# DeepGraphLearning/RNNLogic

Measured on AMD Instinct MI355X. Metric: queries/sec PredictorPlus forward, FB15k-237, 1/2/4/8 GPU; MRR parity, higher is better.
Workload: dtype fp32; 1 GPU; FB15k-237 test split: 1514 batches, 40932 queries, sharded over 1 rank(s) by the reference evaluate()'s DistributedSampler; PredictorPlus(lstm,3,16,sum) + RotatE(D=1000,gamma=9); rnnlogic_rules.txt (131883 rules, L<=3); seeded synthetic train graph and RotatE tables; batch_size=32, parallelism=dp1 (test batches sharded, KG replicated), batches_per_rank=1514

## Files before the change

### include/rnnlogic_hip.h

```cpp
#ifndef RNNLOGIC_HIP_H
#define RNNLOGIC_HIP_H

#include <stddef.h>
#include <stdint.h>

#ifdef __cplusplus
extern "C" {
#endif

#define RNNL_OK 0
#define RNNL_ERR_INVALID 1
#define RNNL_ERR_HIP 2
#define RNNL_ERR_OVERFLOW 3
#define RNNL_ERR_NOMEM 4
#define RNNL_ERR_INTERNAL 5
#define RNNL_ERR_RANGE 6

#define RNNL_AGG_SUM 0
#define RNNL_AGG_PNA 1

#define RNNL_FEATURE_ADD 0
#define RNNL_FEATURE_NONE 1

typedef struct rnnl_graph_s *rnnl_graph;
// ... 85 lines not shown
                             int32_t workgroups, int32_t deferred, void *stream);
int rnnl_forward_status(void *workspace, void *stream);
int rnnl_forward_status_totals(void *workspace, void *stream, int64_t *totals);
int rnnl_forward_header_bytes(size_t *bytes);
int rnnl_forward_status_host(const void *header, int64_t *totals);
#define RNNL_FLAG_MIXED 1
int rnnl_forward_status_flags(void *workspace, void *stream, int64_t *totals, uint32_t *flags);
int rnnl_forward_flags_host(const void *header, uint32_t *flags);
int rnnl_forward_host_info(rnnl_graph g, int32_t *out);
int rnnl_ground(rnnl_graph g, rnnl_rules r, const int64_t *all_h, const int64_t *all_r,
                const int64_t *edges_to_remove, int32_t n_queries, int32_t *n_cand, void *workspace,
                size_t workspace_bytes, int32_t capacity_scale, void *stream);
int rnnl_ground_export_candidates(void *workspace, int32_t n_queries, int32_t capacity_scale, const int32_t *n_cand,
                                  const int64_t *cand_off, int32_t *out_t, int32_t *out_nent, void *stream);
int rnnl_ground_export_entries(void *workspace, int32_t n_queries, int32_t capacity_scale, const int32_t *n_cand,
                               const int64_t *ent_off, int32_t *out_node, int32_t *out_count, void *stream);
int rnnl_debug_profile(void *dev_counters);
int rnnl_debug_clock(void *dev_counters);

int rnnl_debug_capacity(int64_t frontier_base, int64_t contrib_base, int64_t pool_per_query);
int rnnl_debug_sort_bits(int32_t bits);
int rnnl_debug_pair_memo(int32_t on);
int rnnl_debug_dedupe(int32_t min_rows);

int rnnl_linear_node_weights_size(rnnl_rules r, size_t *bytes);
int rnnl_linear_node_weights(rnnl_rules r, const float *rule_weights, int32_t n_rules, void *node_w, void *stream);
int rnnl_predictor_forward(rnnl_graph g, rnnl_rules r, const void *node_w, int32_t feature, const int64_t *all_h,
                           const int64_t *all_r, const int64_t *edges_to_remove, int32_t n_queries, float *score,
                           uint8_t *mask, int32_t *n_cand, void *workspace, size_t workspace_bytes,
                           int32_t capacity_scale, void *stream);
int rnnl_predictor_ground(rnnl_graph g, rnnl_rules r, const int64_t *all_h, const int64_t *all_r,
                          const int64_t *edges_to_remove, int32_t n_queries, int32_t *n_cand, void *workspace,
                          size_t workspace_bytes, int32_t capacity_scale, void *stream);
int rnnl_predictor_score(rnnl_graph g, rnnl_rules r, const void *node_w, int32_t feature, const int64_t *all_h,
                         const int64_t *all_r, int32_t n_queries, float *score, uint8_t *mask, int32_t *n_cand,
                         void *workspace, size_t workspace_bytes, int32_t capacity_scale, void *stream);
int rnnl_predictor_rule_stats(void *workspace, int32_t n_queries, int32_t capacity_scale, const int32_t *n_cand,
                              rnnl_rules r, const int64_t *all_r, const int64_t *all_t, int32_t ld, int64_t *pos,
                              int64_t *tot, void *stream);
int rnnl_predictor_backward(void *workspace, int32_t n_queries, int32_t capacity_scale, const int32_t *n_cand,
                            rnnl_rules r, const int64_t *all_r, int32_t n_entities, const float *grad_score,
                            int32_t ld, double *grad_node, void *stream);

int rnnl_fill_rows(const float *row, int32_t n_queries, int32_t n_entities, float *score, void *stream);
int rnnl_fill_value(float value, int64_t n, float *score, void *stream);

// ... 151 lines not shown
```

### rnnlogic_amd/_native.py

```python
import ctypes
import functools
import os
import subprocess

HERE = os.path.dirname(os.path.abspath(__file__))
LIB_PATH = os.path.join(HERE, "_build", "librnnlogic_hip.so")

RNNL_OK, RNNL_ERR_INVALID, RNNL_ERR_HIP, RNNL_ERR_OVERFLOW, RNNL_ERR_NOMEM, RNNL_ERR_INTERNAL, RNNL_ERR_RANGE = \
    0, 1, 2, 3, 4, 5, 6
AGG_SUM, AGG_PNA = 0, 1
FEATURE_ADD, FEATURE_NONE = 0, 1
ROTATE_DIRECT, ROTATE_MFMA = 0, 1
FLAG_MIXED = 1
ERR_COUNT_WIDTH, ERR_NODE_RANGE, ERR_ACC_RANGE = 8, 16, 32
TOPK_MAX = 1024
KGE_TAIL, KGE_HEAD = 0, 1

_P = ctypes.c_void_p
_I32 = ctypes.c_int32
_I64 = ctypes.c_int64
_F32 = ctypes.c_float

SIGNATURES = [
    ("rnnl_last_error", ctypes.c_char_p, []),
# ... 36 lines not shown
    ("rnnl_forward_host_info", ctypes.c_int, [_P, _P]),
    ("rnnl_forward_header_bytes", ctypes.c_int, [_P]),
    ("rnnl_forward_status_host", ctypes.c_int, [_P, _P]),
    ("rnnl_forward_status_flags", ctypes.c_int, [_P, _P, _P, _P]),
    ("rnnl_forward_flags_host", ctypes.c_int, [_P, _P]),
    ("rnnl_ground", ctypes.c_int, [_P, _P, _P, _P, _P, _I32, _P, _P, ctypes.c_size_t, _I32, _P]),
    ("rnnl_ground_export_candidates", ctypes.c_int, [_P, _I32, _I32, _P, _P, _P, _P, _P]),
    ("rnnl_ground_export_entries", ctypes.c_int, [_P, _I32, _I32, _P, _P, _P, _P, _P]),
    ("rnnl_linear_node_weights_size", ctypes.c_int, [_P, _P]),
    ("rnnl_linear_node_weights", ctypes.c_int, [_P, _P, _I32, _P, _P]),
    ("rnnl_predictor_forward", ctypes.c_int,
     [_P, _P, _P, _I32, _P, _P, _P, _I32, _P, _P, _P, _P, ctypes.c_size_t, _I32, _P]),
    ("rnnl_predictor_ground", ctypes.c_int, [_P, _P, _P, _P, _P, _I32, _P, _P, ctypes.c_size_t, _I32, _P]),
    ("rnnl_predictor_score", ctypes.c_int,
     [_P, _P, _P, _I32, _P, _P, _I32, _P, _P, _P, _P, ctypes.c_size_t, _I32, _P]),
    ("rnnl_predictor_rule_stats", ctypes.c_int, [_P, _I32, _I32, _P, _P, _P, _P, _I32, _P, _P, _P]),
    ("rnnl_predictor_backward", ctypes.c_int, [_P, _I32, _I32, _P, _P, _P, _I32, _P, _I32, _P, _P]),
    ("rnnl_debug_profile", ctypes.c_int, [_P]),
    ("rnnl_debug_clock", ctypes.c_int, [_P]),
    ("rnnl_debug_capacity", ctypes.c_int, [_I64, _I64, _I64]),
    ("rnnl_debug_sort_bits", ctypes.c_int, [_I32]),
    ("rnnl_debug_pair_memo", ctypes.c_int, [_I32]),
    ("rnnl_debug_dedupe", ctypes.c_int, [_I32]),
    ("rnnl_fill_rows", ctypes.c_int, [_P, _I32, _I32, _P, _P]),
    ("rnnl_fill_value", ctypes.c_int, [_F32, _I64, _P, _P]),
    ("rnnl_rotate_table_sizes", ctypes.c_int, [_I32, _I32, _I32, _I32, _P, _P]),
    ("rnnl_rotate_entity_table", ctypes.c_int, [_P, _I32, _I32, _I32, _P, _P]),
    ("rnnl_rotate_relation_table", ctypes.c_int, [_P, _I32, _I32, _F32, _P, _P]),
    ("rnnl_rotate_workspace_size", ctypes.c_int, [_I32, _I32, _I32, _I32, _P]),
    ("rnnl_multi_hot", ctypes.c_int, [_P, _P, _P, _I64, _P, _I32, _I32, _P, _P]),
    ("rnnl_train_batch", ctypes.c_int,
     [_P, _I64, _I32, _P, _P, _P, _I64, _P, _P, _I64, _I32, _P, _P, _P, _P, _P, _P]),
    ("rnnl_filter_flags", ctypes.c_int, [_P, _P, _P, _I64, _P, _I32, _I32, _P, _P]),
    ("rnnl_filtered_ranks", ctypes.c_int, [_P, _P, _P, _P, _I32, _I32, _P, _P, _P]),
    ("rnnl_topk_rows", ctypes.c_int, [_P, _P, _P, _P, _I32, _I32, _I32, _P, _P, _P, _P]),
    ("rnnl_miner_create", ctypes.c_int, [_P, _I64, _I32, _I32, _P]),
    ("rnnl_miner_destroy", ctypes.c_int, [_P]),
    ("rnnl_rule_search", ctypes.c_int, [_P, _I32, _P, _I64, _P, _I64, _P, _P]),
    ("rnnl_miner_set_rules", ctypes.c_int, [_P, _P, _P, _P, _P]),
    ("rnnl_miner_ground_count", ctypes.c_int, [_P, _P, _I64, _I64, _P, _I64, _P, _P, _P]),
    ("rnnl_miner_ground_fill", ctypes.c_int, [_P, _P, _I64, _I64, _P, _I64, _P, _P, _P, _I64, _P, _P]),
    ("rnnl_miner_learn", ctypes.c_int,
     [_P, _P, _I64, _I64, _P, _I64, _P, _P, _P, ctypes.c_double, ctypes.c_double, ctypes.c_double, _I32, _P]),
    ("rnnl_miner_h_score", ctypes.c_int,
     [_P, _P, _I64, _I64, _P, _I64, _P, _P, _P, _I32, ctypes.c_double, ctypes.c_double, _P]),
    ("rnnl_miner_read", ctypes.c_int, [_P, _P, _P, _P]),
# ... 129 lines not shown
```

### rnnlogic_amd/csrc/fwd.h

```cpp
#pragma once
#include <hip/hip_runtime.h>

#include <algorithm>
#include <cstdint>

#include "internal.h"

namespace rnnl {

constexpr int BS = 256;
constexpr int GBS = 256;
constexpr int SOLO_GBS = 512;
constexpr int HBITS = 12;
constexpr int HCAP = 1 << HBITS;
constexpr int OCC_CAP = 1024;
constexpr int WBITS = 11;
constexpr int WIN = 1 << WBITS;
constexpr int MAXE_BITS = 19;
constexpr int SORT_WINS = 256;
constexpr int MAX_SBITS = MAXE_BITS - 8;
static_assert((SORT_WINS << MAX_SBITS) == (1 << MAXE_BITS), "SORT_WINS windows of 2^MAX_SBITS entities hold 2^MAXE_BITS");
static_assert((1 << MAX_SBITS) <= WIN, "a sort window must fit the dense pass's direct map");
constexpr int HB = WIN;
constexpr int HB_LOAD = HB * 3 / 4;
// ... 51 lines not shown
  int32_t sbits;
  float *score;
  uint8_t *mask;
  int32_t *n_cand;
  uint64_t *digest;
  unsigned char *ws;
  int64_t fcap, pcap, pool_cap;
  int32_t nslots;
  unsigned char *slots;
  int64_t *q_base;
  float *q_scale;
  const int32_t *order;
  int32_t atomic_out;
  const int32_t *row_of;
  int4 *cand;
  int2 *bent;
  float *memo;
  unsigned long long *ptab, *ptab_region;
  int32_t psbits, pbr, pbo, pbc, pbc3;
  int2 *chunks;
  int64_t chunk_cap;
  unsigned long long *prof;
};

extern unsigned long long *g_prof;

__device__ __forceinline__ uint64_t mix64(uint64_t x) {
  x += 0x9E3779B97F4A7C15ULL;
  x = (x ^ (x >> 30)) * 0xBF58476D1CE4E5B9ULL;
  x = (x ^ (x >> 27)) * 0x94D049BB133111EBULL;
  return x ^ (x >> 31);
}

__device__ __forceinline__ uint32_t hash32(uint32_t k) { return k * 2654435761u; }

__device__ __forceinline__ int64_t score_index(const KParams &p, int q, int t) {
  return (int64_t)(p.row_of ? p.row_of[q] : q) * p.g.E + t;
}

struct Ent {
  uint32_t k, c;
};

struct Slot {
  Ent *f0;
  int64_t fcap;
// ... 170 lines not shown
    trailer[1] = (unsigned)shift;
    trailer[2] = bad ? 1u : 0u;
  }
  return shift;
}

__device__ __forceinline__ void next_chunks(unsigned int *ctr, long long nchunks, int k, unsigned &c, unsigned &cend) {
  const unsigned long long stat = (unsigned long long)gridDim.x * (BS / 64) * k;
  if (cend == 0u) {
    c = (blockIdx.x * (BS / 64) + (threadIdx.x >> 6)) * (unsigned)k;
  } else if ((long long)stat >= nchunks) {
    c = (unsigned)nchunks;
  } else {
    if ((threadIdx.x & 63) == 0) c = (unsigned)stat + atomicAdd(ctr, (unsigned)k);
    c = __builtin_amdgcn_readfirstlane(c);
  }
  cend = c + (unsigned)k;
}

extern bool g_pair_memo;
void launch_chunk_list(const KParams &p, hipStream_t st);
void launch_ground(const KParams &p, int agg, hipStream_t st, int grid = 0);
void launch_score(const KParams &p, const RulesDev &rl, hipStream_t st, int grid);
int setup_params(const char *who, rnnl_graph g, rnnl_rules r, const int64_t *all_h, const int64_t *all_r,
                 const int64_t *etr, int32_t nq, int32_t *n_cand, void *ws, size_t ws_bytes, int32_t scale,
                 KParams &p);
void set_score_params(KParams &p, const rnnl_predictor_params *pp, float *score, uint8_t *mask, uint64_t *digest);
bool bad_params(const rnnl_predictor_params *pp, const float *score);
KParams export_params(void *ws, int32_t nq, int32_t scale, const int32_t *n_cand);
void plan_enqueue(const Plan &pl, hipStream_t st);
void replicate_enqueue(const Plan &pl, int E, float *score, int32_t *n_cand, hipStream_t st);

}
```

### rnnlogic_amd/csrc/ground.hip

```cpp
#include <hip/hip_runtime.h>

#include <cstdlib>
#include <map>
#include <cstring>
#include <string>

#include "fwd.h"
#include "hostside.h"

namespace rnnl {

unsigned long long *g_prof = nullptr;
int64_t g_fcap_base = FCAP_BASE, g_pcap_base = PCAP_BASE, g_pool_per_query = POOL_PER_QUERY;
int g_sort_bits = -1;

template <int G>
struct __align__(16) SmemT {
  union {
    struct {
      int key[HCAP];
      uint32_t val[HCAP];
    } a;
    struct {
      int map[WIN];
// ... 1252 lines not shown
                              const int64_t *all_r, const int64_t *etr, int32_t nq, int32_t *n_cand, void *ws,
                              size_t ws_bytes, int32_t scale, int32_t workgroups, void *stream) {
  if (aggregator != RNNL_AGG_SUM && aggregator != RNNL_AGG_PNA) {
    set_error("rnnl_predictorplus_ground: bad aggregator");
    return RNNL_ERR_INVALID;
  }
  KParams p;
  if (int rc = setup_params("rnnl_predictorplus_ground", g, r, all_h, all_r, etr, nq, n_cand, ws, ws_bytes, scale,
                            p))
    return rc;
  hipStream_t st = (hipStream_t)stream;
  RNNL_HIP_CHECK(hipMemsetAsync(ws, 0, HDR_WORDS_BYTES, st));
  if (nq == 0) return RNNL_OK;
  p.agg = aggregator;
  launch_ground(p, aggregator, st, workgroups);
  RNNL_HIP_CHECK(hipGetLastError());
  return RNNL_OK;
}

static int score_rows(rnnl_graph g, rnnl_rules r, const rnnl_predictor_params *pp, const int64_t *all_h,
                      const int64_t *all_r, int32_t nq, float *score, uint8_t *mask, int32_t *n_cand,
                      uint64_t *digest, void *ws, size_t ws_bytes, int32_t scale, int32_t workgroups,
                      int32_t deferred, const int32_t *row_of, void *stream) {
  if (bad_params(pp, score) || !n_cand || (deferred != 0 && deferred != 2) ||
      (deferred == 2 && (mask || pp->feature != RNNL_FEATURE_ADD))) {
    set_error("rnnl_predictorplus_score: bad arguments");
    return RNNL_ERR_INVALID;
  }
  KParams p;
  if (int rc = setup_params("rnnl_predictorplus_score", g, r, all_h, all_r, nullptr, nq, n_cand, ws, ws_bytes,
                            scale, p))
    return rc;
  if (nq == 0) return RNNL_OK;
  set_score_params(p, pp, score, mask, digest);
  p.atomic_out = deferred == 2;
  p.row_of = row_of;
  hipStream_t st = (hipStream_t)stream;
  launch_score(p, r->d, st, workgroups);
  RNNL_HIP_CHECK(hipGetLastError());
  return RNNL_OK;
}

int rnnl_predictorplus_score(rnnl_graph g, rnnl_rules r, const rnnl_predictor_params *pp, const int64_t *all_h,
                             const int64_t *all_r, int32_t nq, float *score, uint8_t *mask, int32_t *n_cand,
                             uint64_t *digest, void *ws, size_t ws_bytes, int32_t scale, int32_t workgroups,
                             int32_t deferred, void *stream) {
  return score_rows(g, r, pp, all_h, all_r, nq, score, mask, n_cand, digest, ws, ws_bytes, scale, workgroups, deferred,
                    nullptr, stream);
}

int rnnl_ground(rnnl_graph g, rnnl_rules r, const int64_t *all_h, const int64_t *all_r, const int64_t *etr,
                int32_t nq, int32_t *n_cand, void *ws, size_t ws_bytes, int32_t scale, void *stream) {
  KParams p;
  if (int rc = setup_params("rnnl_ground", g, r, all_h, all_r, etr, nq, n_cand, ws, ws_bytes, scale, p)) return rc;
  hipStream_t st = (hipStream_t)stream;
  RNNL_HIP_CHECK(hipMemsetAsync(ws, 0, HDR_WORDS_BYTES, st));
  if (nq == 0) return RNNL_OK;
  p.agg = RNNL_AGG_SUM;
  launch_ground(p, RNNL_AGG_SUM, st);
  RNNL_HIP_CHECK(hipGetLastError());
  return RNNL_OK;
}

int rnnl_ground_export_candidates(void *ws, int32_t nq, int32_t scale, const int32_t *n_cand,
                                  const int64_t *cand_off, int32_t *out_t, int32_t *out_nent, void *stream) {
  if (!ws || nq < 0 || scale < 1 || !n_cand || !cand_off || !out_t || !out_nent) {
    set_error("rnnl_ground_export_candidates: bad arguments");
    return RNNL_ERR_INVALID;
  }
// ... 13 lines not shown
  }
  if (nq == 0) return RNNL_OK;
  const KParams p = export_params(ws, nq, scale, n_cand);
  hipLaunchKernelGGL(export_entries_kernel, dim3((unsigned)std::min<int64_t>(nq, 4096)), dim3(EXP_BS), 0,
                     (hipStream_t)stream, p, ent_off, out_node, out_count);
  RNNL_HIP_CHECK(hipGetLastError());
  return RNNL_OK;
}

int rnnl_debug_pair_memo(int32_t on) {
  g_pair_memo = on != 0;
  return RNNL_OK;
}

constexpr int32_t DEDUPE_MIN_ROWS = 512;
static int32_t g_dedupe_min = DEDUPE_MIN_ROWS;

int rnnl_debug_dedupe(int32_t min_rows) {
  if (min_rows < -1) {
    set_error("rnnl_debug_dedupe: need min_rows >= 0 (0: off), or -1 for the default");
    return RNNL_ERR_INVALID;
  }
  g_dedupe_min = min_rows < 0 ? DEDUPE_MIN_ROWS : min_rows;
  return RNNL_OK;
}

int rnnl_debug_sort_bits(int32_t bits) {
  g_sort_bits = bits;
  return RNNL_OK;
}

int rnnl_debug_profile(void *dev_counters) {
  g_prof = static_cast<unsigned long long *>(dev_counters);
  return RNNL_OK;
}

int rnnl_debug_capacity(int64_t frontier_base, int64_t contrib_base, int64_t pool_per_query) {
  if (frontier_base <= 0 && contrib_base <= 0 && pool_per_query <= 0) {
    g_fcap_base = FCAP_BASE;
    g_pcap_base = PCAP_BASE;
    g_pool_per_query = POOL_PER_QUERY;
    return RNNL_OK;
  }
  if (frontier_base < 256 || contrib_base < 256 || frontier_base < contrib_base || pool_per_query < 1 ||
      frontier_base > FCAP_BASE || contrib_base > PCAP_BASE || pool_per_query > POOL_PER_QUERY) {
    set_error("rnnl_debug_capacity: need 256 <= contrib <= frontier <= defaults, 1 <= pool <= default");
// ... 158 lines not shown
  pl.ur = reinterpret_cast<int64_t *>(base + Ly.off_ur);
  pl.hkey = reinterpret_cast<unsigned long long *>(base + Ly.off_hkey);
  pl.hrow = reinterpret_cast<unsigned int *>(base + Ly.off_hrow);
  unsigned int *pin_nu = h->pinned + 48;
  RNNL_HIP_CHECK(hipEventRecord(h->in, main));
  RNNL_HIP_CHECK(hipStreamWaitEvent(h->a, h->in, 0));
  plan_enqueue(pl, h->a);
  RNNL_HIP_CHECK(hipGetLastError());
  RNNL_HIP_CHECK(hipMemcpyAsync(pin_nu, pl.hdr, sizeof(unsigned int), hipMemcpyDeviceToHost, h->a));
  RNNL_HIP_CHECK(hipStreamSynchronize(h->a));
  nu = (int32_t)*pin_nu;
  if (nu < 1 || nu > nq) {
    set_error("rnnl_predictorplus_forward_rotate: bad row plan");
    return RNNL_ERR_INTERNAL;
  }
  return RNNL_OK;
}

static int forward_rotate_enqueue(HostSide *h, rnnl_graph g, rnnl_rules r, const rnnl_predictor_params *pp,
                                  const rnnl_rotate_args *rot, const int64_t *all_h, const int64_t *all_r,
                                  const int64_t *etr, int32_t nq, float *score, uint8_t *mask, int32_t *n_cand,
                                  uint64_t *digest, void *ws, size_t ws_bytes, int32_t scale, int32_t ground_wg,
                                  int32_t score_wg, int32_t zeroed, void *const *events, hipStream_t main,
                                  int32_t E, int32_t nq_out, const int32_t *row_of) {
  auto mark = [&](int k) -> hipError_t {
    return events && events[k] ? hipEventRecord((hipEvent_t)events[k], main) : hipSuccess;
  };
  if (!zeroed)
    if (int rc = rnnl_forward_rotate_zero(score, (size_t)nq_out * (size_t)E, main)) return rc;
  RNNL_HIP_CHECK(hipEventRecord(h->in, main));
  RNNL_HIP_CHECK(mark(0));
  RNNL_HIP_CHECK(hipStreamWaitEvent(h->a, h->in, 0));
  RNNL_HIP_CHECK(hipStreamWaitEvent(h->b, h->in, 0));
  if (int rc = rnnl_predictorplus_ground(g, r, pp->aggregator, all_h, all_r, etr, nq, n_cand, ws, ws_bytes, scale,
                                         ground_wg, h->a))
    return rc;
  RNNL_HIP_CHECK(hipStreamWaitEvent(main, h->zero, 0));
  if (int rc = rotate_score_rows(rot->eemb, rot->etab, rot->rtab, rot->dim, rot->gamma, all_h, all_r, nq, E, score, 2,
                                 rot->mode, rot->workspace, rot->workspace_bytes, rot->pieces, rot->first_share,
                                 row_of, main))
    return rc;
  RNNL_HIP_CHECK(mark(1));
  if (mask) {
    RNNL_HIP_CHECK(hipMemsetAsync(mask, 1, (size_t)nq_out * (size_t)E, h->b));
    RNNL_HIP_CHECK(hipEventRecord(h->mask, h->b));
  }
  RNNL_HIP_CHECK(hipStreamWaitEvent(h->a, h->zero, 0));
  if (int rc = score_rows(g, r, pp, all_h, all_r, nq, score, nullptr, n_cand, digest, ws, ws_bytes, scale, score_wg, 2,
                          row_of, h->a))
    return rc;
  RNNL_HIP_CHECK(hipEventRecord(h->side, h->a));
  RNNL_HIP_CHECK(hipStreamWaitEvent(main, h->side, 0));
  if (mask) RNNL_HIP_CHECK(hipStreamWaitEvent(main, h->mask, 0));
  RNNL_HIP_CHECK(mark(2));
  return RNNL_OK;
}

int rnnl_predictorplus_forward_rotate(rnnl_graph g, rnnl_rules r, const rnnl_predictor_params *pp,
                                      const rnnl_rotate_args *rot, const int64_t *all_h, const int64_t *all_r,
                                      const int64_t *etr, int32_t nq, float *score, uint8_t *mask, int32_t *n_cand,
                                      uint64_t *digest, void *ws, size_t ws_bytes, int32_t scale, int32_t ground_wg,
                                      int32_t score_wg, int32_t zeroed, void *const *events, void *stream,
                                      int64_t *totals, uint32_t *flags) {
  if (bad_params(pp, score) || !rot || !n_cand || !ws || nq < 0 || pp->feature != RNNL_FEATURE_ADD) {
    set_error("rnnl_predictorplus_forward_rotate: bad arguments");
    return RNNL_ERR_INVALID;
  }
  if (nq == 0) return RNNL_OK;
  DeviceGuard guard(g->device);
  HostSide *h = overlap_side("rnnl_predictorplus_forward_rotate");
  if (!h) return RNNL_ERR_HIP;
  hipStream_t main = (hipStream_t)stream;
  const int32_t E = rot->n_entities;
  Plan pl{};
  int32_t nu = nq;
  int rc = RNNL_OK;
  hipStreamCaptureStatus cap = hipStreamCaptureStatusNone;
  if (!etr && !digest && g_dedupe_min > 0 && nq >= g_dedupe_min && nq >= 2 && all_h && all_r && g && r &&
      scale >= 1 && hipStreamIsCapturing(main, &cap) == hipSuccess && cap == hipStreamCaptureStatusNone) {
    if (!zeroed) {
      rc = rnnl_forward_rotate_zero(score, (size_t)nq * (size_t)E, main);
      zeroed = 1;
    }
    if (!rc) rc = row_plan(h, g, r, all_h, all_r, nq, ws, ws_bytes, scale, main, pl, nu);
  }
  const bool dedupe = nu < nq;
  if (!rc)
    rc = dedupe ? forward_rotate_enqueue(h, g, r, pp, rot, pl.uh, pl.ur, nullptr, nu, score, mask, pl.n_cand, nullptr,
                                         ws, ws_bytes, scale, ground_wg, score_wg, zeroed, events, main, E, nq,
                                         pl.row_of)
                : forward_rotate_enqueue(h, g, r, pp, rot, all_h, all_r, etr, nq, score, mask, n_cand, digest, ws,
                                         ws_bytes, scale, ground_wg, score_wg, zeroed, events, main, E, nq, nullptr);
  if (!rc && dedupe) {
    replicate_enqueue(pl, E, score, n_cand, main);
    if (hipGetLastError() != hipSuccess) {
      set_error("rnnl_predictorplus_forward_rotate: replicate launch failed");
      rc = RNNL_ERR_HIP;
    }
  }
  if (rc) {
    if (hipEventRecord(h->side, h->a) == hipSuccess) (void)hipStreamWaitEvent(main, h->side, 0);
    if (hipEventRecord(h->mask, h->b) == hipSuccess) (void)hipStreamWaitEvent(main, h->mask, 0);
    (void)hipStreamSynchronize(h->a);
    (void)hipStreamSynchronize(h->b);
    return rc;
  }
  return rnnl_forward_status_flags(ws, main, totals, flags);
}

int rnnl_forward_host_info(rnnl_graph g, int32_t *out) {
  if (!g || !out) {
    set_error("rnnl_forward_host_info: bad arguments");
    return RNNL_ERR_INVALID;
  }
  out[0] = g->device;
// ... 50 lines not shown
```

### rnnlogic_amd/csrc/score.hip

```cpp
#include <hip/hip_runtime.h>

#include "fwd.h"

namespace rnnl {

__device__ __forceinline__ uint32_t rec_off(int n, int stride) { return (uint32_t)n * (uint32_t)stride; }

struct Mlp0Lds {
  uint2 a0[8][2][64];
  float s1w[128], s1b[4];
};

typedef _Float16 f16x4 __attribute__((ext_vector_type(4)));
typedef float f32x4 __attribute__((ext_vector_type(4)));

__device__ __forceinline__ float relu(float x) { return __builtin_amdgcn_fmed3f(x, 0.f, __builtin_huge_valf()); }

__device__ __forceinline__ void split_f16(float v, _Float16 &hi, _Float16 &lo) {
  hi = (_Float16)v;
  lo = (_Float16)(v - (float)hi);
}

__device__ __forceinline__ void load_mlp0(Mlp0Lds &m, const float *__restrict__ W) {
  for (int i = threadIdx.x; i < 128; i += blockDim.x) m.s1w[i] = W[W_S1W + i];
// ... 484 lines not shown
  if (threadIdx.x < 128) s_relb[threadIdx.x] = relation_bias(p, r, threadIdx.x);
  __syncthreads();
  const int shift = (int)reinterpret_cast<const unsigned int *>(p.node_w + (int64_t)p.rl.n_nodes * kStrideSum)[1];
  const float inv_scale = ldexpf(1.f, -shift);
  const int lane = threadIdx.x & 63, wv = threadIdx.x >> 6;
  for (int b0 = wv * 64; b0 < nl; b0 += BS) {
    const int i = b0 + lane;
    const int n = i < nl ? p.rl.head_leaf_node[lp + i] : -1;
    float f[16];
#pragma unroll
    for (int d = 0; d < 16; ++d) f[d] = 0.f;
    if (n >= 0) {
      const int *x = reinterpret_cast<const int *>(p.node_w + rec_off(n, kStrideSum));
#pragma unroll
      for (int d = 0; d < 16; ++d) f[d] = (float)((double)x[d] * (double)inv_scale);
    }
    float x1[16];
    sum_hidden(s_w, f, x1);
    const float out = score_mlp_f16(x1, s_w.m, s_stage[wv], s_relb);
    if (n >= 0) p.memo[n] = out;
  }
}

__device__ __forceinline__ void sum_write_out(const KParams &p, int q, int t, float out, float base) {
  const int64_t idx = score_index(p, q, t);
  if (p.atomic_out) {
    unsafeAtomicAdd(p.score + idx, out);
    return;
  }
  p.score[idx] = p.feature == RNNL_FEATURE_NONE ? out : out + base;
  if (p.mask) p.mask[idx] = 1;
}

__device__ __forceinline__ float sum_base(const KParams &p, int q, int t) {
  if (p.feature == RNNL_FEATURE_NONE || p.atomic_out) return 0.f;
  return p.base_row ? p.base_row[t] : p.score[score_index(p, q, t)];
}

constexpr unsigned long long PAIR_NOKEY = ~0ull;

__device__ __forceinline__ void entry_cswap(unsigned &oa, unsigned &ca, unsigned &ob, unsigned &cb) {
  if (ob < oa || (ob == oa && cb < ca)) {
    const unsigned to = oa, tc = ca;
    oa = ob;
    ca = cb;
    ob = to;
    cb = tc;
  }
}

__device__ __forceinline__ unsigned long long pair_key(const KParams &p, int r, int root, int z, int2 b0, int2 b1,
                                                       int2 b2) {
  unsigned o0 = (unsigned)(b0.x - root), c0 = (unsigned)b0.y;
  unsigned o1 = z >= 2 ? (unsigned)(b1.x - root) : 0u, c1 = z >= 2 ? (unsigned)b1.y : 0u;
  unsigned o2 = z >= 3 ? (unsigned)(b2.x - root) : 0u, c2 = z >= 3 ? (unsigned)b2.y : 0u;
  if (z >= 2) entry_cswap(o0, c0, o1, c1);
  if (z == 3) {
    entry_cswap(o1, c1, o2, c2);
    entry_cswap(o0, c0, o1, c1);
// ... 68 lines not shown
      fp += (uint64_t)cu * p.rl.node_fp[n];
    }
  }
#pragma unroll
  for (int off = 32; off >= 1; off >>= 1) {
#pragma unroll
    for (int d = 0; d < 16; ++d) acc[d] += __shfl_xor(acc[d], off, 64);
    csum += __shfl_xor(csum, off, 64);
    if constexpr (DIGEST) {
      deg += __shfl_xor(deg, off, 64);
      fp += __shfl_xor(fp, off, 64);
    }
  }
  float v = 0.f;
#pragma unroll
  for (int d = 0; d < 16; ++d)
    if (lane == d) v = (float)(acc[d] * (double)inv_scale);
  if (lane < 16) fslot[lane] = v;
}

template <bool DIGEST>
__device__ __forceinline__ void sum_score_lane(const KParams &p, const SumLds &w, const float *relb, float *stage,
                                               bool live, const int2 it, const int4 cr, const float (&f)[16],
                                               long long deg, uint64_t fp, float base, int r, int root) {
  if constexpr (DIGEST)
    if (live)
      atomicAdd(reinterpret_cast<unsigned long long *>(p.digest + it.x),
                (unsigned long long)mix64((uint64_t)cr.x ^ mix64((uint64_t)deg ^ mix64(fp))));
  asm volatile("" ::: "memory");
  float x1[16];
  sum_hidden(w, f, x1);
  const float out = score_mlp_f16(x1, w.m, stage, relb);
  if (!live) return;
  sum_write_out(p, it.x, cr.x, out, base);
  if (!DIGEST && p.ptab && cr.z <= 3) {
    const int2 z0 = make_int2(0, 0);
    const unsigned long long key = pair_key(p, r, root, cr.z, p.bent[cr.y], cr.z >= 2 ? p.bent[cr.y + 1] : z0,
                                            cr.z >= 3 ? p.bent[cr.y + 2] : z0);
    if (key != PAIR_NOKEY) pair_insert(p, key, out);
  }
}

template <bool DIGEST, bool COOP>
__device__ __forceinline__ void sum_chunk_flush(const KParams &p, const SumLds &w, const float *relb, float *stage,
                                                const int2 *queue, int m, float inv_scale, int r, int root,
                                                float *fbig) {
  const int lane = threadIdx.x & 63;
  if constexpr (!COOP) {
    const bool live = lane < m;
    int2 it = make_int2(0, 0);
    int4 cr = make_int4(0, 0, 0, 0);
    float base = 0.f;
    float f[16];
    long long deg = 0;
    uint64_t fp = 0;
#pragma unroll
    for (int d = 0; d < 16; ++d) f[d] = 0.f;
    if (live) {
      it = queue[lane];
      cr = p.cand[it.y];
      base = sum_base(p, it.x, cr.x);
      gather_sum<DIGEST>(p, cr.y, cr.z, inv_scale, f, deg, fp);
    }
    sum_score_lane<DIGEST>(p, w, relb, stage, live, it, cr, f, deg, fp, base, r, root);
    return;
  }
  int2 it = make_int2(0, 0);
  int4 cr = make_int4(0, 0, 0, 0);
  if (lane < m) {
    it = queue[lane];
    cr = p.cand[it.y];
  }
  bool todo = lane < m;
#pragma unroll 1
  while (true) {
    uint64_t big = __ballot(todo && cr.z > BIG_ENTRIES);
    int slot = -1;
    long long bdeg = 0;
    uint64_t bfp = 0;
#pragma unroll 1
    for (int nb = 0; big && nb < BIG_SLOTS; ++nb) {
      const int owner = __builtin_ctzll(big);
      big &= big - 1;
      const int beg = __builtin_amdgcn_readlane(cr.y, owner), cnt = __builtin_amdgcn_readlane(cr.z, owner);
      uint64_t csum;
      long long deg;
      uint64_t fp;
// ... 3 lines not shown
        bdeg = deg;
        bfp = fp;
      }
    }
    wave_lds_sync();
    const bool go = todo && (cr.z <= BIG_ENTRIES || slot != -1);
    float base = 0.f;
    float f[16];
    long long deg = 0;
    uint64_t fp = 0;
#pragma unroll
    for (int d = 0; d < 16; ++d) f[d] = 0.f;
    if (go) {
      base = sum_base(p, it.x, cr.x);
      if (slot >= 0) {
#pragma unroll
        for (int d = 0; d < 16; ++d) f[d] = fbig[slot * 16 + d];
        deg = bdeg;
        fp = bfp;
      } else {
        gather_sum<DIGEST>(p, cr.y, cr.z, inv_scale, f, deg, fp);
      }
    }
    sum_score_lane<DIGEST>(p, w, relb, stage, go, it, cr, f, deg, fp, base, r, root);
    if (go) todo = false;
    wave_lds_sync();
    if (__ballot(todo) == 0ull) break;
  }
}

constexpr int SUM_CK = 8;
#ifndef RNNL_OVERLAP_WPE
#define RNNL_OVERLAP_WPE 5
#endif
#ifndef RNNL_OVERLAP_COOP
#define RNNL_OVERLAP_COOP true
#endif
constexpr int SOLO_FEW_ROWS = 8192;
#ifndef RNNL_FEW_WPE
#define RNNL_FEW_WPE 4
#endif
#ifndef RNNL_SMALL_WPE
#define RNNL_SMALL_WPE 4
#endif
#ifndef RNNL_SMALL_OVERLAP_WPE
#define RNNL_SMALL_OVERLAP_WPE 4
#endif
// ... 52 lines not shown
      wave_lds_sync();
      relb[lane] = relation_bias(p, r, lane);
      relb[lane + 64] = relation_bias(p, r, lane + 64);
      cur_r = r;
      cur_root = __builtin_amdgcn_readfirstlane(p.rl.head_root[r]);
    }
    const int nc = p.n_cand[q];
    const int64_t qb = p.q_base[q];
    const int s = s0 + lane;
    bool queued = false;
    if (s < nc) {
      const int4 cr = p.cand[qb + s];
      queued = true;
      unsigned long long key = PAIR_NOKEY;
      if (cr.z == 1) {
        const int2 be = p.bent[cr.y];
        if (be.y == 1 && p.memo) {
          queued = false;
          const float base = sum_base(p, q, cr.x);
          if constexpr (DIGEST)
            atomicAdd(reinterpret_cast<unsigned long long *>(p.digest + q),
                      (unsigned long long)mix64((uint64_t)cr.x ^ mix64((uint64_t)p.rl.node_nrules[be.x] ^
                                                                        mix64(p.rl.node_fp[be.x]))));
          sum_write_out(p, q, cr.x, p.memo[be.x], base);
        } else if (!DIGEST && p.ptab) {
          key = pair_key(p, r, cur_root, 1, be, make_int2(0, 0), make_int2(0, 0));
        }
      } else if (!DIGEST && p.ptab && cr.z <= 3) {
        key = pair_key(p, r, cur_root, cr.z, p.bent[cr.y], p.bent[cr.y + 1],
                       cr.z == 3 ? p.bent[cr.y + 2] : make_int2(0, 0));
      }
      float out;
      if (key != PAIR_NOKEY && pair_lookup(p, key, out)) {
        queued = false;
        sum_write_out(p, q, cr.x, out, sum_base(p, q, cr.x));
      }
    }
    const uint64_t bal = __ballot(queued);
    const int pos = n + (int)__builtin_amdgcn_mbcnt_hi((uint32_t)(bal >> 32),
                                                       __builtin_amdgcn_mbcnt_lo((uint32_t)bal, 0u));
    wave_lds_sync();
    if (queued) queue[pos] = make_int2(q, (int)(qb + s));
    n += (int)__popcll(bal);
    ++c;
  }
}

bool g_pair_memo = true;

__global__ void pack_weights_kernel(KParams p, float *__restrict__ W) {
  const int kin = p.agg == RNNL_AGG_SUM ? 16 : 192;
  for (int i = blockIdx.x * blockDim.x + threadIdx.x; i < W_FLOATS; i += gridDim.x * blockDim.x) {
    float v = 0.f;
    if (i < W_ADDB) {
      if (i < 16 * kin) v = p.add_w[i];
    } else if (i < W_LNW) {
      v = p.add_b[i - W_ADDB];
    } else if (i < W_LNB) {
// ... 53 lines not shown
  }
  const bool small = nq <= MEMO_SCAN_ROWS;
  if (small && pair)
    p.memo = nullptr;
  else
    hipLaunchKernelGGL(memo_sum_kernel, dim3((unsigned)std::max(p.g.R, 1)), dim3(BS), 0, st, p, W);
  if (p.digest && small)
    hipLaunchKernelGGL((score_sum_chunk_kernel<true, true, 8>), dim3(cgrid), dim3(BS), 0, st, p, W);
  else if (p.digest)
    hipLaunchKernelGGL((score_sum_chunk_kernel<true, false, 8>), dim3(cgrid), dim3(BS), 0, st, p, W);
  else if (p.atomic_out && small)
    hipLaunchKernelGGL((score_sum_chunk_kernel<false, true, RNNL_SMALL_OVERLAP_WPE>), dim3(cgrid), dim3(BS), 0, st, p,
                       W);
  else if (p.atomic_out)
    hipLaunchKernelGGL((score_sum_chunk_kernel<false, RNNL_OVERLAP_COOP, RNNL_OVERLAP_WPE>), dim3(cgrid), dim3(BS), 0, st, p, W);
  else if (small)
    hipLaunchKernelGGL((score_sum_chunk_kernel<false, true, RNNL_SMALL_WPE>), dim3(cgrid), dim3(BS), 0, st, p, W);
  else if (nq <= SOLO_FEW_ROWS)
    hipLaunchKernelGGL((score_sum_chunk_kernel<false, false, RNNL_FEW_WPE>), dim3(cgrid), dim3(BS), 0, st, p, W);
  else
    hipLaunchKernelGGL((score_sum_chunk_kernel<false, RNNL_SOLO_COOP, RNNL_SOLO_WPE>), dim3(cgrid), dim3(BS), 0, st, p, W);
}

}
```

### rnnlogic_amd/predictors.py

```python
import collections
import ctypes
import logging
import math

import numpy as np
import torch
import torch.nn as nn

from . import _native
from .data import _DeviceHandle
from .embedding import RotatE
from .layers import MLP, FuncToNode, FuncToNodeSum


def _read_rules(input):
    rules = []
    if isinstance(input, list):
        for rule in input:
            rules.append((rule[0], list(rule[1:])))
    elif isinstance(input, str):
        with open(input, "r") as fi:
            for line in fi:
                tok = line.strip().split()
                if tok and "." in tok[-1]:
# ... 1065 lines not shown
        else:
            raise NotImplementedError
        self.relation_emb = torch.nn.Embedding(self.num_relations, self.hidden_dim)
        self.score_model = MLP(self.hidden_dim * 2, [128, 1])
        if entity_feature == "bias":
            self.bias = torch.nn.parameter.Parameter(torch.zeros(self.num_entities))
        elif entity_feature == "RotatE":
            self.RotatE = RotatE(embedding_path)
        self._native_rules = {}
        self._node_cache = {}
        self._tok_cache = {}
        self._ws = {}
        self._ws_chunks = {}
        self._side = {}
        self._ws_uses = {}
        self._flags = np.zeros(1, dtype=np.uint32)
        self.capacity_scale = 1
        self.overlap = True
        self.overlap_ground_wg = 128
        self.overlap_score_wg = 128 if aggregator == "sum" else 384
        self.zero_early = aggregator != "sum"
        self.ground_early = True
        self.native_dedupe_min = None
        self.rotate_yield = True
        self.rotate_share = 0.8
        self.fused_backward = True
        self._pf = {}
        self.prefetch_depth = 2
        self.encoder_trie = True
        self.prefetch_dropped = 0

    def set_rules(self, input):
        self.rules = _read_rules(input)
        logging.info("Predictor+: read {} rules from {}.".format(len(self.rules),
                                                                "list" if isinstance(input, list) else "file"))
        self.num_rules = len(self.rules)
        self.max_length = max([len(rule[1]) for rule in self.rules])
        self.relation2rules = [[] for _ in range(self.num_relations)]
        for index, rule in enumerate(self.rules):
            self.relation2rules[rule[0]].append([index, rule])
        self.rule_features = torch.tensor(
            [[h] + b + [self.padding_index] * (self.max_length - len(b)) for h, b in self.rules], dtype=torch.long)
        self._max_rules_per_relation = max(len(x) for x in self.relation2rules)
        if self.type == "emb":
            self.rule_emb = nn.parameter.Parameter(torch.zeros(self.num_rules, self.hidden_dim))
            nn.init.kaiming_uniform_(self.rule_emb, a=math.sqrt(5), mode="fan_in")
# ... 184 lines not shown
        if not self.fused:
            with torch.no_grad():
                score, mask, n_cand = self.forward_coo(all_h, all_r, etr)
            return (score, mask, n_cand) if return_ncand else (score, mask)
        try:
            return self._forward_rows_fused(device, all_h, all_r, etr, nq, return_ncand, digest, events)
        except _native.NativeError as e:
            if e.code != _native.RNNL_ERR_RANGE or digest is not None:
                raise
        logging.info("PredictorPlus: %s; rows recomputed on the grounding COO (int64 counts, fp32 torch ops)",
                     _native.lib().rnnl_last_error().decode(errors="replace"))
        with torch.no_grad():
            score, mask, n_cand = self.forward_coo(all_h, all_r, etr, nonfinite=True)
        return (score, mask, n_cand) if return_ncand else (score, mask)

    def _forward_rows_fused(self, device, all_h, all_r, etr, nq, return_ncand, digest, events):
        g = self.graph.device_graph(device)
        nr = self.native_rules(device)
        rec = (lambda k: events.setdefault(k, torch.cuda.Event(enable_timing=True)).record()) \
            if events is not None else (lambda k: None)
        rec("start")
        score = torch.empty((nq, self.num_entities), dtype=torch.float32, device=device)
        overlap = self.entity_feature == "RotatE" and self.overlap and nq >= 2
        if overlap and self.zero_early:
            _native.call("rnnl_forward_rotate_zero", score.data_ptr(), score.numel(),
                         torch.cuda.current_stream(device).cuda_stream)
        early = None
        if not overlap and self.ground_early and events is None and nq >= 2:
            main = torch.cuda.current_stream(device)
            side = self._ground_stream(device)
            scale = self.capacity_scale
            ws = self._workspace(device, nq, scale)
            n_cand = torch.empty(nq, dtype=torch.int32, device=device)
            side.wait_stream(main)
            _native.call("rnnl_predictorplus_ground", g, nr.ptr,
                         _native.AGG_SUM if self.aggregator == "sum" else _native.AGG_PNA, all_h.data_ptr(),
                         all_r.data_ptr(), etr.data_ptr() if etr is not None else None, nq, n_cand.data_ptr(),
                         ws.data_ptr(), ws.numel(), scale, 0, side.cuda_stream)
            early = (side, ws, scale)
        node_w = self.node_weights(device)
        params, keep = self._params(device, node_w)
        stream = torch.cuda.current_stream(device).cuda_stream
        none_mode = params.feature == _native.FEATURE_NONE
        if early is None:
            n_cand = torch.empty(nq, dtype=torch.int32, device=device)
        if overlap:
            mask = self._forward_overlap(device, g, nr, params, all_h, all_r, etr, score, n_cand, digest, events)
# ... 40 lines not shown

    def _ground_stream(self, device):
        key = ("ground_stream", self._device_index(device))
        st = self._side.get(key)
        if st is None:
            st = self._side[key] = torch.cuda.Stream(device)
        return st

    def _overlap_workspace(self, device, nq, scale):
        sk = ("need", self._device_index(device), nq, scale)
        need = self._ws_chunks.get(sk)
        if need is None:
            need = ctypes.c_size_t()
            _native.call("rnnl_forward_workspace_size", self.graph.device_graph(device),
                         self.native_rules(device).ptr, nq, scale, ctypes.byref(need))
            self._ws_chunks[sk] = need
        key = self._device_index(device)
        ws = self._ws_chunks.get(key)
        if ws is None or ws.numel() < need.value:
            ws = torch.empty(need.value, dtype=torch.uint8, device=device)
            self._ws_chunks[key] = ws
        return ws

    def _forward_overlap(self, device, g, nr, params, all_h, all_r, etr, score, n_cand, digest, events):
        main = torch.cuda.current_stream(device)
        nq = all_h.numel()
        pieces = 2 if self.rotate_yield and params.aggregator == _native.AGG_PNA else 1
        rot = self.RotatE.native_args(nq, pieces, self.rotate_share if pieces > 1 else 0.0)
        mask = torch.empty((nq, self.num_entities), dtype=torch.bool, device=device)
        ev = None
        if events is not None:
            evs = [events.setdefault(k, torch.cuda.Event(enable_timing=True)) for k in ("base", "ground", "end")]
            for e in evs:
                e.record(main)
            ev = (ctypes.c_void_p * 3)(*[e.cuda_event for e in evs])
        zeroed = 1 if self.zero_early else 0
        while True:
            scale = self.capacity_scale
            ws = self._overlap_workspace(device, nq, scale)
            if self.native_dedupe_min is not None:
                _native.call("rnnl_debug_dedupe", int(self.native_dedupe_min))
            rc = _native.lib().rnnl_predictorplus_forward_rotate(
                g, nr.ptr, ctypes.byref(params), ctypes.byref(rot), all_h.data_ptr(), all_r.data_ptr(),
                etr.data_ptr() if etr is not None else None, nq, score.data_ptr(), mask.data_ptr(), n_cand.data_ptr(),
                digest.data_ptr() if digest is not None else None, ws.data_ptr(), ws.numel(), scale,
                self.overlap_ground_wg, self.overlap_score_wg, zeroed, ev, main.cuda_stream, None,
                self._flags.ctypes.data_as(ctypes.c_void_p))
            if self.native_dedupe_min is not None:
                _native.call("rnnl_debug_dedupe", -1)
            if rc == _native.RNNL_ERR_OVERFLOW and self.capacity_scale < 64:
                self.capacity_scale *= 2
                zeroed = 0
                logging.info("PredictorPlus: workspace overflow, capacity_scale -> %d", self.capacity_scale)
                continue
            _native.check(rc)
            return mask

    @_native.on_input_device
    def forward_autograd(self, all_h, all_r, edges_to_remove, query_r=None):
        device = all_h.device
        all_h = all_h.to(torch.int64)
        all_r = all_r.to(torch.int64)
        nq, E = all_h.numel(), self.num_entities
        if self.fused and self.aggregator == "sum" and self.fused_backward and device.type == "cuda":
            try:
                return self._forward_sum_train(all_h, all_r, edges_to_remove, query_r)
            except _native.NativeError as e:
                if e.code != _native.RNNL_ERR_RANGE:
                    raise
        if self.fused and self.aggregator == "pna" and self.fused_backward and device.type == "cuda":
            try:
                return self._forward_pna_train(all_h, all_r, edges_to_remove, query_r)
# ... 273 lines not shown
```

Baseline: 973,300 queries/s.

## Write RotatE scores directly and add rule scores via candidate slots

For the sum aggregator, the forward pass no longer zeroes the full nq×E score matrix and accumulates into it with atomics. RotatE now writes scores directly. The rule-scoring kernel stores each candidate's score in a spare slot of the candidate record, and a new finish kernel adds those values into the score matrix after both streams join. This removes a large memset and the atomic read-modify-writes, and lets RotatE start without waiting on the zero event. The cost is an extra kernel launch and serialisation of the finish step after both branches.

```diff
diff --git a/include/rnnlogic_hip.h b/include/rnnlogic_hip.h
--- a/include/rnnlogic_hip.h
+++ b/include/rnnlogic_hip.h
@@ -131,6 +131,7 @@
 int rnnl_debug_sort_bits(int32_t bits);
 int rnnl_debug_pair_memo(int32_t on);
 int rnnl_debug_dedupe(int32_t min_rows);
+int rnnl_debug_written_once(int32_t on);
 
 int rnnl_linear_node_weights_size(rnnl_rules r, size_t *bytes);
 int rnnl_linear_node_weights(rnnl_rules r, const float *rule_weights, int32_t n_rules, void *node_w, void *stream);
diff --git a/rnnlogic_amd/_native.py b/rnnlogic_amd/_native.py
--- a/rnnlogic_amd/_native.py
+++ b/rnnlogic_amd/_native.py
@@ -82,6 +82,7 @@
     ("rnnl_debug_sort_bits", ctypes.c_int, [_I32]),
     ("rnnl_debug_pair_memo", ctypes.c_int, [_I32]),
     ("rnnl_debug_dedupe", ctypes.c_int, [_I32]),
+    ("rnnl_debug_written_once", ctypes.c_int, [_I32]),
     ("rnnl_fill_rows", ctypes.c_int, [_P, _I32, _I32, _P, _P]),
     ("rnnl_fill_value", ctypes.c_int, [_F32, _I64, _P, _P]),
     ("rnnl_rotate_table_sizes", ctypes.c_int, [_I32, _I32, _I32, _I32, _P, _P]),
diff --git a/rnnlogic_amd/csrc/fwd.h b/rnnlogic_amd/csrc/fwd.h
--- a/rnnlogic_amd/csrc/fwd.h
+++ b/rnnlogic_amd/csrc/fwd.h
@@ -97,6 +97,8 @@
   int64_t chunk_cap;
   unsigned long long *prof;
 };
+
+enum { OUT_DIRECT = 0, OUT_ATOMIC = 1, OUT_SLOT = 2 };
 
 extern unsigned long long *g_prof;
 
@@ -313,6 +315,7 @@
 void launch_chunk_list(const KParams &p, hipStream_t st);
 void launch_ground(const KParams &p, int agg, hipStream_t st, int grid = 0);
 void launch_score(const KParams &p, const RulesDev &rl, hipStream_t st, int grid);
+void launch_sum_finish(const KParams &p, hipStream_t st);
 int setup_params(const char *who, rnnl_graph g, rnnl_rules r, const int64_t *all_h, const int64_t *all_r,
                  const int64_t *etr, int32_t nq, int32_t *n_cand, void *ws, size_t ws_bytes, int32_t scale,
                  KParams &p);
diff --git a/rnnlogic_amd/csrc/ground.hip b/rnnlogic_amd/csrc/ground.hip
--- a/rnnlogic_amd/csrc/ground.hip
+++ b/rnnlogic_amd/csrc/ground.hip
@@ -1298,8 +1298,9 @@
                       const int64_t *all_r, int32_t nq, float *score, uint8_t *mask, int32_t *n_cand,
                       uint64_t *digest, void *ws, size_t ws_bytes, int32_t scale, int32_t workgroups,
                       int32_t deferred, const int32_t *row_of, void *stream) {
-  if (bad_params(pp, score) || !n_cand || (deferred != 0 && deferred != 2) ||
-      (deferred == 2 && (mask || pp->feature != RNNL_FEATURE_ADD))) {
+  if (bad_params(pp, score) || !n_cand || (deferred != 0 && deferred != 2 && deferred != 3) ||
+      (deferred && (mask || pp->feature != RNNL_FEATURE_ADD)) ||
+      (deferred == 3 && pp->aggregator != RNNL_AGG_SUM)) {
     set_error("rnnl_predictorplus_score: bad arguments");
     return RNNL_ERR_INVALID;
   }
@@ -1309,7 +1310,7 @@
     return rc;
   if (nq == 0) return RNNL_OK;
   set_score_params(p, pp, score, mask, digest);
-  p.atomic_out = deferred == 2;
+  p.atomic_out = deferred == 3 ? OUT_SLOT : deferred == 2 ? OUT_ATOMIC : OUT_DIRECT;
   p.row_of = row_of;
   hipStream_t st = (hipStream_t)stream;
   launch_score(p, r->d, st, workgroups);
@@ -1317,10 +1318,29 @@
   return RNNL_OK;
 }
 
+static int finish_rows(rnnl_graph g, rnnl_rules r, const int64_t *all_h, const int64_t *all_r, int32_t nq, float *score,
+                       int32_t *n_cand, void *ws, size_t ws_bytes, int32_t scale, const int32_t *row_of,
+                       void *stream) {
+  KParams p;
+  if (int rc = setup_params("rnnl_predictorplus_forward_rotate", g, r, all_h, all_r, nullptr, nq, n_cand, ws, ws_bytes,
+                            scale, p))
+    return rc;
+  p.score = score;
+  p.row_of = row_of;
+  p.atomic_out = OUT_SLOT;
+  launch_sum_finish(p, (hipStream_t)stream);
+  RNNL_HIP_CHECK(hipGetLastError());
+  return RNNL_OK;
+}
+
 int rnnl_predictorplus_score(rnnl_graph g, rnnl_rules r, const rnnl_predictor_params *pp, const int64_t *all_h,
                              const int64_t *all_r, int32_t nq, float *score, uint8_t *mask, int32_t *n_cand,
                              uint64_t *digest, void *ws, size_t ws_bytes, int32_t scale, int32_t workgroups,
                              int32_t deferred, void *stream) {
+  if (deferred == 3) {
+    set_error("rnnl_predictorplus_score: bad arguments");
+    return RNNL_ERR_INVALID;
+  }
   return score_rows(g, r, pp, all_h, all_r, nq, score, mask, n_cand, digest, ws, ws_bytes, scale, workgroups, deferred,
                     nullptr, stream);
 }
@@ -1380,6 +1400,13 @@
     return RNNL_ERR_INVALID;
   }
   g_dedupe_min = min_rows < 0 ? DEDUPE_MIN_ROWS : min_rows;
+  return RNNL_OK;
+}
+
+static bool g_written_once = true;
+
+int rnnl_debug_written_once(int32_t on) {
+  g_written_once = on != 0;
   return RNNL_OK;
 }
 
@@ -1584,11 +1611,11 @@
                                   const int64_t *etr, int32_t nq, float *score, uint8_t *mask, int32_t *n_cand,
                                   uint64_t *digest, void *ws, size_t ws_bytes, int32_t scale, int32_t ground_wg,
                                   int32_t score_wg, int32_t zeroed, void *const *events, hipStream_t main,
-                                  int32_t E, int32_t nq_out, const int32_t *row_of) {
+                                  int32_t E, int32_t nq_out, const int32_t *row_of, bool once) {
   auto mark = [&](int k) -> hipError_t {
     return events && events[k] ? hipEventRecord((hipEvent_t)events[k], main) : hipSuccess;
   };
-  if (!zeroed)
+  if (!zeroed && !once)
     if (int rc = rnnl_forward_rotate_zero(score, (size_t)nq_out * (size_t)E, main)) return rc;
   RNNL_HIP_CHECK(hipEventRecord(h->in, main));
   RNNL_HIP_CHECK(mark(0));
@@ -1597,22 +1624,24 @@
   if (int rc = rnnl_predictorplus_ground(g, r, pp->aggregator, all_h, all_r, etr, nq, n_cand, ws, ws_bytes, scale,
                                          ground_wg, h->a))
     return rc;
-  RNNL_HIP_CHECK(hipStreamWaitEvent(main, h->zero, 0));
-  if (int rc = rotate_score_rows(rot->eemb, rot->etab, rot->rtab, rot->dim, rot->gamma, all_h, all_r, nq, E, score, 2,
-                                 rot->mode, rot->workspace, rot->workspace_bytes, rot->pieces, rot->first_share,
-                                 row_of, main))
+  if (!once || zeroed) RNNL_HIP_CHECK(hipStreamWaitEvent(main, h->zero, 0));
+  if (int rc = rotate_score_rows(rot->eemb, rot->etab, rot->rtab, rot->dim, rot->gamma, all_h, all_r, nq, E, score,
+                                 once ? 0 : 2, rot->mode, rot->workspace, rot->workspace_bytes, rot->pieces,
+                                 rot->first_share, row_of, main))
     return rc;
   RNNL_HIP_CHECK(mark(1));
   if (mask) {
     RNNL_HIP_CHECK(hipMemsetAsync(mask, 1, (size_t)nq_out * (size_t)E, h->b));
     RNNL_HIP_CHECK(hipEventRecord(h->mask, h->b));
   }
-  RNNL_HIP_CHECK(hipStreamWaitEvent(h->a, h->zero, 0));
-  if (int rc = score_rows(g, r, pp, all_h, all_r, nq, score, nullptr, n_cand, digest, ws, ws_bytes, scale, score_wg, 2,
-                          row_of, h->a))
+  if (!once) RNNL_HIP_CHECK(hipStreamWaitEvent(h->a, h->zero, 0));
+  if (int rc = score_rows(g, r, pp, all_h, all_r, nq, score, nullptr, n_cand, digest, ws, ws_bytes, scale, score_wg,
+                          once ? 3 : 2, row_of, h->a))
     return rc;
   RNNL_HIP_CHECK(hipEventRecord(h->side, h->a));
   RNNL_HIP_CHECK(hipStreamWaitEvent(main, h->side, 0));
+  if (once)
+    if (int rc = finish_rows(g, r, all_h, all_r, nq, score, n_cand, ws, ws_bytes, scale, row_of, main)) return rc;
   if (mask) RNNL_HIP_CHECK(hipStreamWaitEvent(main, h->mask, 0));
   RNNL_HIP_CHECK(mark(2));
   return RNNL_OK;
@@ -1634,13 +1663,14 @@
   if (!h) return RNNL_ERR_HIP;
   hipStream_t main = (hipStream_t)stream;
   const int32_t E = rot->n_entities;
+  const bool once = g_written_once && pp->aggregator == RNNL_AGG_SUM;
   Plan pl{};
   int32_t nu = nq;
   int rc = RNNL_OK;
   hipStreamCaptureStatus cap = hipStreamCaptureStatusNone;
   if (!etr && !digest && g_dedupe_min > 0 && nq >= g_dedupe_min && nq >= 2 && all_h && all_r && g && r &&
       scale >= 1 && hipStreamIsCapturing(main, &cap) == hipSuccess && cap == hipStreamCaptureStatusNone) {
-    if (!zeroed) {
+    if (!zeroed && !once) {
       rc = rnnl_forward_rotate_zero(score, (size_t)nq * (size_t)E, main);
       zeroed = 1;
     }
@@ -1650,9 +1680,10 @@
   if (!rc)
     rc = dedupe ? forward_rotate_enqueue(h, g, r, pp, rot, pl.uh, pl.ur, nullptr, nu, score, mask, pl.n_cand, nullptr,
                                          ws, ws_bytes, scale, ground_wg, score_wg, zeroed, events, main, E, nq,
-                                         pl.row_of)
+                                         pl.row_of, once)
                 : forward_rotate_enqueue(h, g, r, pp, rot, all_h, all_r, etr, nq, score, mask, n_cand, digest, ws,
-                                         ws_bytes, scale, ground_wg, score_wg, zeroed, events, main, E, nq, nullptr);
+                                         ws_bytes, scale, ground_wg, score_wg, zeroed, events, main, E, nq, nullptr,
+                                         once);
   if (!rc && dedupe) {
     replicate_enqueue(pl, E, score, n_cand, main);
     if (hipGetLastError() != hipSuccess) {
diff --git a/rnnlogic_amd/csrc/score.hip b/rnnlogic_amd/csrc/score.hip
--- a/rnnlogic_amd/csrc/score.hip
+++ b/rnnlogic_amd/csrc/score.hip
@@ -530,7 +530,11 @@
   }
 }
 
-__device__ __forceinline__ void sum_write_out(const KParams &p, int q, int t, float out, float base) {
+__device__ __forceinline__ void sum_write_out(const KParams &p, int q, int t, int64_t ci, float out, float base) {
+  if (p.atomic_out == OUT_SLOT) {
+    reinterpret_cast<float *>(p.cand + ci)[3] = out;
+    return;
+  }
   const int64_t idx = score_index(p, q, t);
   if (p.atomic_out) {
     unsafeAtomicAdd(p.score + idx, out);
@@ -543,6 +547,22 @@
 __device__ __forceinline__ float sum_base(const KParams &p, int q, int t) {
   if (p.feature == RNNL_FEATURE_NONE || p.atomic_out) return 0.f;
   return p.base_row ? p.base_row[t] : p.score[score_index(p, q, t)];
+}
+
+__global__ __launch_bounds__(BS) void sum_finish_kernel(KParams p) {
+  const long long nchunks =
+      (long long)*reinterpret_cast<const unsigned long long *>(reinterpret_cast<const unsigned int *>(p.ws) + H_CHUNKS);
+  const int lane = threadIdx.x & 63;
+  for (long long c = (long long)blockIdx.x * (BS / 64) + (threadIdx.x >> 6); c < nchunks;
+       c += (long long)gridDim.x * (BS / 64)) {
+    const int2 ck = p.chunks[c];
+    const int s = ck.y + lane;
+    if (s < p.n_cand[ck.x]) {
+      const int4 cr = p.cand[p.q_base[ck.x] + s];
+      const int64_t idx = score_index(p, ck.x, cr.x);
+      p.score[idx] = p.score[idx] + __int_as_float(cr.w);
+    }
+  }
 }
 
 constexpr unsigned long long PAIR_NOKEY = ~0ull;
@@ -657,7 +677,8 @@
 template <bool DIGEST>
 __device__ __forceinline__ void sum_score_lane(const KParams &p, const SumLds &w, const float *relb, float *stage,
                                                bool live, const int2 it, const int4 cr, const float (&f)[16],
-                                               long long deg, uint64_t fp, float base, int r, int root) {
+                                               long long deg, uint64_t fp, float base, int r, int root,
+                                               const int2 *queue) {
   if constexpr (DIGEST)
     if (live)
       atomicAdd(reinterpret_cast<unsigned long long *>(p.digest + it.x),
@@ -667,7 +688,7 @@
   sum_hidden(w, f, x1);
   const float out = score_mlp_f16(x1, w.m, stage, relb);
   if (!live) return;
-  sum_write_out(p, it.x, cr.x, out, base);
+  sum_write_out(p, it.x, cr.x, p.atomic_out == OUT_SLOT ? queue[threadIdx.x & 63].y : 0, out, base);
   if (!DIGEST && p.ptab && cr.z <= 3) {
     const int2 z0 = make_int2(0, 0);
     const unsigned long long key = pair_key(p, r, root, cr.z, p.bent[cr.y], cr.z >= 2 ? p.bent[cr.y + 1] : z0,
@@ -697,7 +718,7 @@
       base = sum_base(p, it.x, cr.x);
       gather_sum<DIGEST>(p, cr.y, cr.z, inv_scale, f, deg, fp);
     }
-    sum_score_lane<DIGEST>(p, w, relb, stage, live, it, cr, f, deg, fp, base, r, root);
+    sum_score_lane<DIGEST>(p, w, relb, stage, live, it, cr, f, deg, fp, base, r, root, queue);
     return;
   }
   int2 it = make_int2(0, 0);
@@ -747,7 +768,7 @@
         gather_sum<DIGEST>(p, cr.y, cr.z, inv_scale, f, deg, fp);
       }
     }
-    sum_score_lane<DIGEST>(p, w, relb, stage, go, it, cr, f, deg, fp, base, r, root);
+    sum_score_lane<DIGEST>(p, w, relb, stage, go, it, cr, f, deg, fp, base, r, root, queue);
     if (go) todo = false;
     wave_lds_sync();
     if (__ballot(todo) == 0ull) break;
@@ -846,7 +867,7 @@
             atomicAdd(reinterpret_cast<unsigned long long *>(p.digest + q),
                       (unsigned long long)mix64((uint64_t)cr.x ^ mix64((uint64_t)p.rl.node_nrules[be.x] ^
                                                                         mix64(p.rl.node_fp[be.x]))));
-          sum_write_out(p, q, cr.x, p.memo[be.x], base);
+          sum_write_out(p, q, cr.x, qb + s, p.memo[be.x], base);
         } else if (!DIGEST && p.ptab) {
           key = pair_key(p, r, cur_root, 1, be, make_int2(0, 0), make_int2(0, 0));
         }
@@ -857,7 +878,7 @@
       float out;
       if (key != PAIR_NOKEY && pair_lookup(p, key, out)) {
         queued = false;
-        sum_write_out(p, q, cr.x, out, sum_base(p, q, cr.x));
+        sum_write_out(p, q, cr.x, qb + s, out, sum_base(p, q, cr.x));
       }
     }
     const uint64_t bal = __ballot(queued);
@@ -957,4 +978,9 @@
     hipLaunchKernelGGL((score_sum_chunk_kernel<false, RNNL_SOLO_COOP, RNNL_SOLO_WPE>), dim3(cgrid), dim3(BS), 0, st, p, W);
 }
 
-}
+void launch_sum_finish(const KParams &p, hipStream_t st) {
+  const unsigned grid = (unsigned)std::min<int64_t>(std::max<int64_t>(p.nq, 1), NUM_CU * SCORE_WG_PER_CU);
+  hipLaunchKernelGGL(sum_finish_kernel, dim3(grid), dim3(BS), 0, st, p);
+}
+
+}
diff --git a/rnnlogic_amd/predictors.py b/rnnlogic_amd/predictors.py
--- a/rnnlogic_amd/predictors.py
+++ b/rnnlogic_amd/predictors.py
@@ -1111,6 +1111,7 @@
         self.zero_early = aggregator != "sum"
         self.ground_early = True
         self.native_dedupe_min = None
+        self.written_once = None
         self.rotate_yield = True
         self.rotate_share = 0.8
         self.fused_backward = True
@@ -1341,7 +1342,8 @@
         rec("start")
         score = torch.empty((nq, self.num_entities), dtype=torch.float32, device=device)
         overlap = self.entity_feature == "RotatE" and self.overlap and nq >= 2
-        if overlap and self.zero_early:
+        once = self.aggregator == "sum" and self.written_once is not False
+        if overlap and self.zero_early and not once:
             _native.call("rnnl_forward_rotate_zero", score.data_ptr(), score.numel(),
                          torch.cuda.current_stream(device).cuda_stream)
         early = None
@@ -1428,6 +1430,12 @@
             self._ws_chunks[key] = ws
         return ws
 
+    def _overlap_knobs(self, on):
+        if self.native_dedupe_min is not None:
+            _native.call("rnnl_debug_dedupe", int(self.native_dedupe_min) if on else -1)
+        if self.written_once is not None:
+            _native.call("rnnl_debug_written_once", int(bool(self.written_once)) if on else 1)
+
     def _forward_overlap(self, device, g, nr, params, all_h, all_r, etr, score, n_cand, digest, events):
         main = torch.cuda.current_stream(device)
         nq = all_h.numel()
@@ -1440,20 +1448,19 @@
             for e in evs:
                 e.record(main)
             ev = (ctypes.c_void_p * 3)(*[e.cuda_event for e in evs])
-        zeroed = 1 if self.zero_early else 0
+        once = params.aggregator == _native.AGG_SUM and self.written_once is not False
+        zeroed = 1 if self.zero_early and not once else 0
         while True:
             scale = self.capacity_scale
             ws = self._overlap_workspace(device, nq, scale)
-            if self.native_dedupe_min is not None:
-                _native.call("rnnl_debug_dedupe", int(self.native_dedupe_min))
+            self._overlap_knobs(True)
             rc = _native.lib().rnnl_predictorplus_forward_rotate(
                 g, nr.ptr, ctypes.byref(params), ctypes.byref(rot), all_h.data_ptr(), all_r.data_ptr(),
                 etr.data_ptr() if etr is not None else None, nq, score.data_ptr(), mask.data_ptr(), n_cand.data_ptr(),
                 digest.data_ptr() if digest is not None else None, ws.data_ptr(), ws.numel(), scale,
                 self.overlap_ground_wg, self.overlap_score_wg, zeroed, ev, main.cuda_stream, None,
                 self._flags.ctypes.data_as(ctypes.c_void_p))
-            if self.native_dedupe_min is not None:
-                _native.call("rnnl_debug_dedupe", -1)
+            self._overlap_knobs(False)
             if rc == _native.RNNL_ERR_OVERFLOW and self.capacity_scale < 64:
                 self.capacity_scale *= 2
                 zeroed = 0
```

Result: no change. 978,900 queries/s, median of 6 (+0.6%).
